# bostoncleek/ergodic_exploration

Hardware: AMD Instinct MI355X
Metric: receding-horizon optimisations/sec at K=10x10, T=200; 1/2/4/8-GPU agent-batch (higher is better)
Workload: dtype f64; 1 GPU; BASELINE configs[3]: 4096-agent batch per GPU, simple_cart, two-Gaussian 12x6 m map, K=10x10, T=200 steps (dt 0.1, horizon 20), n_mem=0; agents_per_gpu=4096, num_basis=10, horizon_steps=200, kinematics=simple_cart, agent_groups=2, steps_per_launch=50, parallelism=agent-batch x1

## Files before the change

### ergodic_exploration_amd/csrc/control_wave_impl.hpp

```cpp
#ifndef EEA_CONTROL_WAVE_HELPERS_HPP
#define EEA_CONTROL_WAVE_HELPERS_HPP

#include <type_traits>

#include "common.hpp"

#ifndef EEA_WSTAMP
#define EEA_WSTAMP(n) ((void)0)
#define EEA_WSTAMP_RT(n) ((void)0)
#define EEA_WSTAMP_HWID(n) ((void)0)
#endif

namespace eea
{
namespace wave
{
constexpr int kMaxS = 4;
constexpr int kStageRows = 32;
constexpr int kRow1 = 68;
constexpr int kTailScratch = 24;

__host__ __device__ constexpr int tab_stride(int K) { return (K + 1) & ~1; }
__host__ __device__ constexpr int park_elems() { return 2 * kMaxS * kWave; }
__host__ __device__ constexpr int d_elems(int K) { return (K * K + 3) & ~3; }
__host__ __device__ constexpr int tile_elems(int K)
// ... 118 lines not shown
{
  if constexpr (NB == 3) {
    asm volatile("s_waitcnt lgkmcnt(0)" : "+v"(qa[0]), "+v"(qa[1]), "+v"(qa[2]), "+v"(qb[0]), "+v"(qb[1]), "+v"(qb[2]));
  } else {
    static_assert(NB == 2, "lean packed instances: K = 5 or 10");
    asm volatile("s_waitcnt lgkmcnt(0)" : "+v"(qa[0]), "+v"(qa[1]), "+v"(qb[0]), "+v"(qb[1]));
  }
}

template <int N>
__device__ __forceinline__ double add_row_ror(double v)
{
  return v + dpp_or_zero<0x120 + N, 0xf>(v);
}

template <typename R, int MODEL>
__device__ __forceinline__ void model_xy(R vx, R vy, R c, R s, R& fx, R& fy)
{
  if (MODEL == kModelOmni) {
    fx = vx * c - vy * s;
    fy = vx * s + vy * c;
  } else {
    fx = vx * c;
    fy = vx * s;
  }
}

template <typename R>
__device__ __forceinline__ R wrap_pi_fast(R rad)
{
  const R pi = static_cast<R>(kPi), two_pi = static_cast<R>(2.0 * kPi);
  const R q = floor((rad + pi) * static_cast<R>(1.0 / (2.0 * kPi)));
  rad = (rad + pi) - q * two_pi;
  if (rad < R(0)) rad += two_pi;
  if (rad >= two_pi) rad -= two_pi;
  return rad - pi;
}

constexpr int waves_per_simd(int KC, int real_size)
{
  return (KC == 20) ? (real_size == 8 ? 2 : 4) : ((KC <= 10 || real_size == 4) ? 4 : 3);
}
constexpr int grad_block(int KC) { return KC; }

}
}
#endif

namespace eea
{
namespace wave
{
template <typename R, int MODEL, int KC, bool STAGES, int WPB, bool RESIDENT = false>
__global__ __launch_bounds__(WPB* kWave, waves_per_simd(KC, sizeof(R))) void control_wave_kernel(
    const ControlParams<R> p_arg, const unsigned B, const int S_arg, const int rollout_arg)
{
  (void)p_arg;
  extern __shared__ __attribute__((aligned(16))) char smem_raw[];
// ... 195 lines not shown
      sincospi_r(th_pre0 * inv_pi, &s, &c);
    }
    bool small = true;
#pragma unroll
    for (int j = 0; j < kMaxS; ++j) small = small && (fabs(dt * (R(0.5) * w[j]) * inv_pi) <= R(0.0625));
    const bool fast_h = sizeof(R) == 8 && __all(small);
    R rx = R(0), ry = R(0);
#pragma unroll
    for (int j = 0; j < kMaxS; ++j) {
      incx[j] = incy[j] = R(0);
      if (j < S) {
        R sm_, cm, cpost, spost;
        if (fast_h) {
          R sd, cd;
          sincospi_small(dt * (R(0.5) * w[j]) * inv_pi, &sd, &cd);
          cm = c * cd - s * sd;
          sm_ = s * cd + c * sd;
          cpost = cm * cd - sm_ * sd;
          spost = sm_ * cd + cm * sd;
        } else {
          const R th_pre = (j == 0) ? thp[0] - dt6 * (((w[0] + R(2) * w[0]) + R(2) * w[0]) + w[0]) : thp[j - 1];
          sincospi_r((th_pre + dt * (R(0.5) * w[j])) * inv_pi, &sm_, &cm);
          const R c2m = R(1) - R(2) * sm_ * sm_, s2m = R(2) * sm_ * cm;
          cpost = c2m * c + s2m * s;
          spost = s2m * c - c2m * s;
        }
        R k1x, k1y, k2x, k2y, k4x, k4y;
        model_xy<R, MODEL>(vx[j], vy[j], c, s, k1x, k1y);
        model_xy<R, MODEL>(vx[j], vy[j], cm, sm_, k2x, k2y);
        model_xy<R, MODEL>(vx[j], vy[j], cpost, spost, k4x, k4y);
        incx[j] = dt6 * (((k1x + R(2) * k2x) + R(2) * k2x) + k4x);
        incy[j] = dt6 * (((k1y + R(2) * k2y) + R(2) * k2y) + k4y);
        rx += incx[j];
        ry += incy[j];
        s_cp[j * kWave + lane] = cpost;
        s_sp[j * kWave + lane] = spost;
        c = cpost;
        s = spost;
      }
      px[j] = rx;
      py[j] = ry;
    }
    const R ix = wave_inclusive_scan_dpp(rx), iy = wave_inclusive_scan_dpp(ry);
    const R bx = x0 + (ix - rx), by = y0 + (iy - ry);
#pragma unroll
    for (int j = 0; j < kMaxS; ++j) {
      px[j] += bx;
// ... 18 lines not shown
  R c1x[kMaxS], s1x[kMaxS], c1y[kMaxS], s1y[kMaxS], g0[kMaxS], g1[kMaxS];
  bool small_b = true;
#pragma unroll
  for (int j = 1; j < kMaxS; ++j) {
    small_b = small_b && (fabs(incx[j] * p.inv_lx) <= R(0.0625)) && (fabs(incy[j] * p.inv_ly) <= R(0.0625));
  }
  const bool fast_b = sizeof(R) == 8 && __all(small_b);
#pragma unroll
  for (int j = 0; j < kMaxS; ++j) {
    c1x[j] = s1x[j] = c1y[j] = s1y[j] = g0[j] = g1[j] = R(0);
    if (j < S) {
      const R x = px[j] - map_x, y = py[j] - map_y;
      if (j > 0 && fast_b) {
        R sd, cd;
        sincospi_small(incx[j] * p.inv_lx, &sd, &cd);
        c1x[j] = c1x[j - 1] * cd - s1x[j - 1] * sd;
        s1x[j] = s1x[j - 1] * cd + c1x[j - 1] * sd;
        sincospi_small(incy[j] * p.inv_ly, &sd, &cd);
        c1y[j] = c1y[j - 1] * cd - s1y[j - 1] * sd;
        s1y[j] = s1y[j - 1] * cd + c1y[j - 1] * sd;
      } else {
        sincospi_r(x * p.inv_lx, &s1x[j], &c1x[j]);
        sincospi_r(y * p.inv_ly, &s1y[j], &c1y[j]);
      }
      const R eps = R(0.05), weight2 = R(50);
      g0[j] = (fmax(x - (p.lx - eps), R(0)) + fmin(x - eps, R(0))) * weight2;
      g1[j] = (fmax(y - (p.ly - eps), R(0)) + fmin(y - eps, R(0))) * weight2;
    }
  }

  EEA_WSTAMP(4);
  int nmem = 0;
  if (p.mem_cols != nullptr) {
    nmem = RESIDENT ? res_nmem : (p.n_mem != nullptr) ? p.n_mem[b] : static_cast<int>(p.mem_stride);
    nmem = nmem < 0 ? 0 : (nmem > static_cast<int>(p.mem_stride) ? static_cast<int>(p.mem_stride) : nmem);
// ... 510 lines not shown
    for (int t = 0; t < NT * NT; ++t) {
#pragma unroll
      for (int r = 0; r < 4; ++r) {
        const int k1 = 16 * (t / NT) + M::row(lane, r);
        const int k2 = 16 * (t % NT) + mi;
        if (k1 < K && k2 < K) {
          R c = invN * (*accs[t])[r];
          if (use_shared) c = shared_ck_value(p, shared_ck, ck_shared_step, k2 * K + k1, c);
          s_D[k2 * K + k1] = lam[t][r] * (c - phi[t][r]);
        }
      }
    }
    lds_fence();
  }

  EEA_WSTAMP(6);
  constexpr int KA = (KC == 16) ? 16 : KC;
  if (!STAGES) {
#pragma unroll
    for (int j = 0; j < kMaxS; ++j) {
      if (j < S) {
        s_g[(2 * j + 0) * kWave + lane] = g0[j];
        s_g[(2 * j + 1) * kWave + lane] = g1[j];
      }
    }
  }
  R ex[STAGES ? kMaxS : 1], ey[STAGES ? kMaxS : 1];
  constexpr bool kCoopTail = sizeof(R) == 8 && (KC == 10 || KC == 5);
  const bool coop_tail = kCoopTail && top_heavy && S == kMaxS;
  constexpr bool kPairGrad = sizeof(R) == 4 && (KC == 20 || KC == 10);
  if constexpr (kPairGrad) {
    typedef float f2 __attribute__((ext_vector_type(2)));
    auto splat = [](float v) { return f2{ v, v }; };
    int zoff = 0;
    asm volatile("" : "+s"(zoff));
    const R* const s_Dz = s_D + zoff;
    auto d_pair = [&](int k2, int k1) { return *reinterpret_cast<const f2*>(((k1 & 2) ? s_Dz : s_D) + k2 * K + k1); };
#pragma unroll
    for (int jp = 0; jp < kMaxS; jp += 2) {
      if (STAGES) ex[jp] = ey[jp] = ex[jp + 1] = ey[jp + 1] = R(0);
      asm volatile("" ::: "memory");
      __builtin_amdgcn_sched_barrier(0);
// ... 67 lines not shown
              ex[j] = exj;
              ey[j] = eyj;
            } else {
              const bool act = j < cnt;
              g0[j] = act ? exj + s_g[(2 * j + 0) * kWave + lane] : R(0);
              g1[j] = act ? eyj + s_g[(2 * j + 1) * kWave + lane] : R(0);
            }
          }
        }
      }
    }
  }
#pragma unroll
  for (int j = 0; j < kMaxS; ++j) {
    if (kPairGrad) break;
    if (STAGES) ex[j] = ey[j] = R(0);
    asm volatile("" ::: "memory");
    __builtin_amdgcn_sched_barrier(0);
    if (j < S && !(j == kMaxS - 1 && coop_tail)) {
      constexpr int KB = grad_block(KC);
      R accx = R(0), accy = R(0);
      const R twox = c1x[j] + c1x[j], twoy = c1y[j] + c1y[j];
      R ta = R(1), tb = c1x[j];
      R ua = R(0), ub = R(1);
#pragma unroll
      for (int kb0 = 0; kb0 < KA; kb0 += KB) {
        if (kb0 > 0) {
          asm volatile("" ::: "memory");
          __builtin_amdgcn_sched_barrier(0);
        }
        R cxa[KB], G[KB];
#pragma unroll
        for (int i = 0; i < KB; ++i) {
          cxa[i] = ta;
          const R tn = twox * tb - ta;
          ta = tb;
          tb = tn;
        }
        {
        {
          const R* const row = s_D + kb0;
#pragma unroll
          for (int i = 0; i < KB; ++i) {
            const int k1 = kb0 + i;
            G[i] = (k1 == 0 || k1 >= KA) ? R(0) : ((kGenericK && k1 >= K) ? R(0) : row[i]);
          }
        }
        R um = R(0), u0 = R(1);
        R tm = R(1), t0 = c1y[j];
#pragma unroll
        for (int k2 = 1; k2 < KA; ++k2) {
          if (!kRowGuard || k2 < K) {
            const R* const row = s_D + k2 * K + kb0;
            R h = R(0);
// ... 17 lines not shown
          }
        }
        }
#pragma unroll
        for (int i = 0; i < KB; ++i) {
          const int k1 = kb0 + i;
          if (k1 > 0 && k1 < KA) accx = fma_k(ua * G[i], k1, accx);
          const R un = twox * ub - ua;
          ua = ub;
          ub = un;
        }
      }
      const R sx = s1x[j], sy = s1y[j];
      const R exj = (-p.pi_lx * sx * accx) * p.expl_weight;
      const R eyj = (-p.pi_ly * sy * accy) * p.expl_weight;
      if (STAGES) {
        ex[j] = exj;
        ey[j] = eyj;
      } else {
        const bool act = j < cnt;
        g0[j] = act ? exj + s_g[(2 * j + 0) * kWave + lane] : R(0);
        g1[j] = act ? eyj + s_g[(2 * j + 1) * kWave + lane] : R(0);
      }
    }
  }
  if constexpr (kCoopTail) {
    if (coop_tail) {
      constexpr int jt = kMaxS - 1;
      asm volatile("" ::: "memory");
      __builtin_amdgcn_sched_barrier(0);
      const int st = lane >> 3, sub = lane & 7;
      R* const s_tail = s_g + 2 * kMaxS * kWave;
      if (lane < 8) {
        s_tail[lane] = c1x[jt];
        s_tail[8 + lane] = c1y[jt];
        s_tail[16 + lane] = s1y[jt];
      }
// ... 58 lines not shown
      px += dpp_or_zero<0xB1, 0xf>(px);
      py += dpp_or_zero<0xB1, 0xf>(py);
      px += dpp_or_zero<0x4E, 0xf>(px);
      py += dpp_or_zero<0x4E, 0xf>(py);
      px += dpp_or_zero<0x141, 0xf>(px);
      py += dpp_or_zero<0x141, 0xf>(py);
      if (sub == 0) {
        s_tail[2 * st] = px;
        s_tail[2 * st + 1] = py;
      }
      lds_fence();
      const R accx = s_tail[2 * (lane & 7)], accy = s_tail[2 * (lane & 7) + 1];
      const R sx = s1x[jt];
      const R exj = (-p.pi_lx * sx * accx) * p.expl_weight;
      const R eyj = (-p.pi_ly * accy) * p.expl_weight;
      if (STAGES) {
        ex[jt] = exj;
        ey[jt] = eyj;
      } else {
        const bool act = jt < cnt;
        g0[jt] = act ? exj + s_g[(2 * jt + 0) * kWave + lane] : R(0);
        g1[jt] = act ? eyj + s_g[(2 * jt + 1) * kWave + lane] : R(0);
      }
    }
  }
  if (STAGES) {
#pragma unroll
    for (int j = 0; j < kMaxS; ++j) {
      if (j < cnt) {
        if (p.edx != nullptr) {
          R* const o = p.edx + 3 * (static_cast<size_t>(T) * b + i0 + j);
          o[0] = ex[j];
          o[1] = ey[j];
          o[2] = R(0);
        }
        if (p.bdx != nullptr) {
          R* const o = p.bdx + 3 * (static_cast<size_t>(T) * b + i0 + j);
          o[0] = g0[j];
          o[1] = g1[j];
          o[2] = R(0);
        }
      }
    }
  }

  EEA_WSTAMP(7);
  R vxr[kMaxS], vyr[kMaxS];
  {
    size_t opaque = 0;
    asm volatile("" : "+v"(opaque));
    const R* const ut_again = ut + opaque;
#pragma unroll
    for (int j = 0; j < kMaxS; ++j) {
      const int src = i0 + j + 1;
      const bool ok = j < cnt && src < T;
      const int idx = ok ? 3 * src : 0;
      const R a = ut_again[idx];
      vxr[j] = ok ? a : R(0);
      vyr[j] = R(0);
      if (MODEL == kModelOmni) {
        const R bq = ut_again[idx + 1];
        vyr[j] = ok ? bq : R(0);
      }
    }
  }
  R r0[kMaxS], r1[kMaxS];
  R tot0, tot1, tot2;
  {
    R s0 = R(0), s1 = R(0);
#pragma unroll
    for (int j = kMaxS - 1; j >= 0; --j) {
      if (STAGES) {
        const bool act = j < cnt;
        g0[j] = act ? ex[j] + g0[j] : R(0);
        g1[j] = act ? ey[j] + g1[j] : R(0);
      }
      s0 += dt * g0[j];
      s1 += dt * g1[j];
      r0[j] = s0;
      r1[j] = s1;
    }
    const R i0s = wave_inclusive_scan_dpp(s0), i1s = wave_inclusive_scan_dpp(s1);
    tot0 = read_lane63(i0s);
    tot1 = read_lane63(i1s);
    const R o0 = tot0 - i0s, o1 = tot1 - i1s;
#pragma unroll
    for (int j = 0; j < kMaxS; ++j) {
// ... 103 lines not shown
```

Measured before the change: 182.0 million optimisations/s.

## Hold D coefficient matrix in registers and broadcast via DPP in gradient

For f64 with K=10 or 5, the Fourier coefficient matrix D is loaded once from LDS into a few VGPRs per lane. The per-step gradient contraction then reads it through hand-written v_fmac_f64_dpp row_newbcast assembly instead of repeated LDS row reads. The edx/bdx stores are also moved into the per-slot loop, and explicit FMA helpers are applied to the RK4 rotation and basis recurrences. The aim is to cut LDS traffic and latency in the gradient loop, at the cost of extra registers, fragile inline asm with manual s_nop hazards, and slightly different rounding from the FMAs.

```diff
diff --git a/ergodic_exploration_amd/csrc/control_wave_impl.hpp b/ergodic_exploration_amd/csrc/control_wave_impl.hpp
--- a/ergodic_exploration_amd/csrc/control_wave_impl.hpp
+++ b/ergodic_exploration_amd/csrc/control_wave_impl.hpp
@@ -9,6 +9,9 @@
 #define EEA_WSTAMP(n) ((void)0)
 #define EEA_WSTAMP_RT(n) ((void)0)
 #define EEA_WSTAMP_HWID(n) ((void)0)
+#endif
+#ifndef EEA_WAVE_REGD
+#define EEA_WAVE_REGD 1
 #endif
 
 namespace eea
@@ -157,6 +160,19 @@
   return v + dpp_or_zero<0x120 + N, 0xf>(v);
 }
 
+template <typename R>
+__device__ __forceinline__ R mul_sub(R a, R b, R c, R d)
+{
+  if constexpr (sizeof(R) == 8) return __builtin_fma(a, b, -(c * d));
+  else return a * b - c * d;
+}
+template <typename R>
+__device__ __forceinline__ R mul_add(R a, R b, R c, R d)
+{
+  if constexpr (sizeof(R) == 8) return __builtin_fma(a, b, c * d);
+  else return a * b + c * d;
+}
+
 template <typename R, int MODEL>
 __device__ __forceinline__ void model_xy(R vx, R vy, R c, R s, R& fx, R& fy)
 {
@@ -168,6 +184,29 @@
     fy = vx * s;
   }
 }
+template <int MODEL>
+__device__ __forceinline__ void model_xy_pinned(double vx, double vy, double c, double s, double& fx, double& fy)
+{
+  if (MODEL == kModelOmni) {
+    fx = mul_sub(vx, c, vy, s);
+    fy = mul_add(vx, s, vy, c);
+  } else {
+    fx = vx * c;
+    fy = vx * s;
+  }
+}
+template <int MODEL>
+__device__ __forceinline__ void model_xy_plus(double vx, double vy, double c, double s, double ax, double ay, double& fx,
+                                              double& fy)
+{
+  if (MODEL == kModelOmni) {
+    fx = mul_sub(vx, c, vy, s) + ax;
+    fy = mul_add(vx, s, vy, c) + ay;
+  } else {
+    fx = __builtin_fma(vx, c, ax);
+    fy = __builtin_fma(vx, s, ay);
+  }
+}
 
 template <typename R>
 __device__ __forceinline__ R wrap_pi_fast(R rad)
@@ -185,6 +224,8 @@
   return (KC == 20) ? (real_size == 8 ? 2 : 4) : ((KC <= 10 || real_size == 4) ? 4 : 3);
 }
 constexpr int grad_block(int KC) { return KC; }
+
+#include "control_wave_regd.inc"
 
 }
 }
@@ -410,23 +451,32 @@
         if (fast_h) {
           R sd, cd;
           sincospi_small(dt * (R(0.5) * w[j]) * inv_pi, &sd, &cd);
-          cm = c * cd - s * sd;
-          sm_ = s * cd + c * sd;
-          cpost = cm * cd - sm_ * sd;
-          spost = sm_ * cd + cm * sd;
+          cm = mul_sub(c, cd, s, sd);
+          sm_ = mul_add(c, sd, s, cd);
+          cpost = mul_sub(cm, cd, sm_, sd);
+          spost = mul_add(sm_, cd, cm, sd);
         } else {
           const R th_pre = (j == 0) ? thp[0] - dt6 * (((w[0] + R(2) * w[0]) + R(2) * w[0]) + w[0]) : thp[j - 1];
           sincospi_r((th_pre + dt * (R(0.5) * w[j])) * inv_pi, &sm_, &cm);
           const R c2m = R(1) - R(2) * sm_ * sm_, s2m = R(2) * sm_ * cm;
-          cpost = c2m * c + s2m * s;
-          spost = s2m * c - c2m * s;
-        }
-        R k1x, k1y, k2x, k2y, k4x, k4y;
-        model_xy<R, MODEL>(vx[j], vy[j], c, s, k1x, k1y);
-        model_xy<R, MODEL>(vx[j], vy[j], cm, sm_, k2x, k2y);
-        model_xy<R, MODEL>(vx[j], vy[j], cpost, spost, k4x, k4y);
-        incx[j] = dt6 * (((k1x + R(2) * k2x) + R(2) * k2x) + k4x);
-        incy[j] = dt6 * (((k1y + R(2) * k2y) + R(2) * k2y) + k4y);
+          cpost = mul_add(s2m, s, c2m, c);
+          spost = mul_sub(s2m, c, c2m, s);
+        }
+        if constexpr (sizeof(R) == 8) {
+          double k2x, k2y, k4x, k4y, k12x, k12y;
+          model_xy_pinned<MODEL>(vx[j], vy[j], cm, sm_, k2x, k2y);
+          model_xy_pinned<MODEL>(vx[j], vy[j], cpost, spost, k4x, k4y);
+          model_xy_plus<MODEL>(vx[j], vy[j], c, s, k2x + k2x, k2y + k2y, k12x, k12y);
+          incx[j] = dt6 * ((k12x + R(2) * k2x) + k4x);
+          incy[j] = dt6 * ((k12y + R(2) * k2y) + k4y);
+        } else {
+          R k1x, k1y, k2x, k2y, k4x, k4y;
+          model_xy<R, MODEL>(vx[j], vy[j], c, s, k1x, k1y);
+          model_xy<R, MODEL>(vx[j], vy[j], cm, sm_, k2x, k2y);
+          model_xy<R, MODEL>(vx[j], vy[j], cpost, spost, k4x, k4y);
+          incx[j] = dt6 * (((k1x + R(2) * k2x) + R(2) * k2x) + k4x);
+          incy[j] = dt6 * (((k1y + R(2) * k2y) + R(2) * k2y) + k4y);
+        }
         rx += incx[j];
         ry += incy[j];
         s_cp[j * kWave + lane] = cpost;
@@ -475,11 +525,12 @@
       if (j > 0 && fast_b) {
         R sd, cd;
         sincospi_small(incx[j] * p.inv_lx, &sd, &cd);
-        c1x[j] = c1x[j - 1] * cd - s1x[j - 1] * sd;
-        s1x[j] = s1x[j - 1] * cd + c1x[j - 1] * sd;
+        constexpr bool kFuseSCdX = (KC == 20), kFuseSCdY = (KC == 20 || KC == 5);
+        c1x[j] = mul_sub(c1x[j - 1], cd, s1x[j - 1], sd);
+        s1x[j] = kFuseSCdX ? mul_add(s1x[j - 1], cd, c1x[j - 1], sd) : mul_add(c1x[j - 1], sd, s1x[j - 1], cd);
         sincospi_small(incy[j] * p.inv_ly, &sd, &cd);
-        c1y[j] = c1y[j - 1] * cd - s1y[j - 1] * sd;
-        s1y[j] = s1y[j - 1] * cd + c1y[j - 1] * sd;
+        c1y[j] = mul_sub(c1y[j - 1], cd, s1y[j - 1], sd);
+        s1y[j] = kFuseSCdY ? mul_add(s1y[j - 1], cd, c1y[j - 1], sd) : mul_add(c1y[j - 1], sd, s1y[j - 1], cd);
       } else {
         sincospi_r(x * p.inv_lx, &s1x[j], &c1x[j]);
         sincospi_r(y * p.inv_ly, &s1y[j], &c1y[j]);
@@ -1020,9 +1071,34 @@
     lds_fence();
   }
 
+  constexpr bool kRegD = EEA_WAVE_REGD && sizeof(R) == 8 && (KC == 10 || KC == 5);
+  constexpr int kDRegs = kRegD ? (KC * KC + 15) / 16 : 1;
+  double Dv[kDRegs];
+  if constexpr (kRegD) {
+#pragma unroll
+    for (int q = 0; q < kDRegs; ++q) Dv[q] = s_D[min(16 * q + (lane & 15), KC * KC - 1)];
+  }
+
   EEA_WSTAMP(6);
   constexpr int KA = (KC == 16) ? 16 : KC;
-  if (!STAGES) {
+  constexpr bool kSumInSlot = !STAGES || kRegD;
+  auto store_edx_bdx = [&](int j, R exj, R eyj, R bx, R by) {
+    if (j < cnt) {
+      if (p.edx != nullptr) {
+        R* const o = p.edx + 3 * (static_cast<size_t>(T) * b + i0 + j);
+        o[0] = exj;
+        o[1] = eyj;
+        o[2] = R(0);
+      }
+      if (p.bdx != nullptr) {
+        R* const o = p.bdx + 3 * (static_cast<size_t>(T) * b + i0 + j);
+        o[0] = bx;
+        o[1] = by;
+        o[2] = R(0);
+      }
+    }
+  };
+  if (kSumInSlot) {
 #pragma unroll
     for (int j = 0; j < kMaxS; ++j) {
       if (j < S) {
@@ -1031,7 +1107,7 @@
       }
     }
   }
-  R ex[STAGES ? kMaxS : 1], ey[STAGES ? kMaxS : 1];
+  R ex[kSumInSlot ? 1 : kMaxS], ey[kSumInSlot ? 1 : kMaxS];
   constexpr bool kCoopTail = sizeof(R) == 8 && (KC == 10 || KC == 5);
   const bool coop_tail = kCoopTail && top_heavy && S == kMaxS;
   constexpr bool kPairGrad = sizeof(R) == 4 && (KC == 20 || KC == 10);
@@ -1129,7 +1205,7 @@
 #pragma unroll
   for (int j = 0; j < kMaxS; ++j) {
     if (kPairGrad) break;
-    if (STAGES) ex[j] = ey[j] = R(0);
+    if (!kSumInSlot) ex[j] = ey[j] = R(0);
     asm volatile("" ::: "memory");
     __builtin_amdgcn_sched_barrier(0);
     if (j < S && !(j == kMaxS - 1 && coop_tail)) {
@@ -1152,7 +1228,9 @@
           ta = tb;
           tb = tn;
         }
-        {
+        if constexpr (kRegD) {
+          RegDGrad<kRegD ? KC : 5>::run(Dv, cxa, G, c1y[j], twoy, accy);
+        } else {
         {
           const R* const row = s_D + kb0;
 #pragma unroll
@@ -1200,13 +1278,15 @@
       const R sx = s1x[j], sy = s1y[j];
       const R exj = (-p.pi_lx * sx * accx) * p.expl_weight;
       const R eyj = (-p.pi_ly * sy * accy) * p.expl_weight;
-      if (STAGES) {
+      if (!kSumInSlot) {
         ex[j] = exj;
         ey[j] = eyj;
       } else {
         const bool act = j < cnt;
-        g0[j] = act ? exj + s_g[(2 * j + 0) * kWave + lane] : R(0);
-        g1[j] = act ? eyj + s_g[(2 * j + 1) * kWave + lane] : R(0);
+        const R bx = s_g[(2 * j + 0) * kWave + lane], by = s_g[(2 * j + 1) * kWave + lane];
+        if (STAGES) store_edx_bdx(j, exj, eyj, bx, by);
+        g0[j] = act ? exj + bx : R(0);
+        g1[j] = act ? eyj + by : R(0);
       }
     }
   }
@@ -1295,34 +1375,21 @@
       const R sx = s1x[jt];
       const R exj = (-p.pi_lx * sx * accx) * p.expl_weight;
       const R eyj = (-p.pi_ly * accy) * p.expl_weight;
-      if (STAGES) {
+      if (!kSumInSlot) {
         ex[jt] = exj;
         ey[jt] = eyj;
       } else {
         const bool act = jt < cnt;
-        g0[jt] = act ? exj + s_g[(2 * jt + 0) * kWave + lane] : R(0);
-        g1[jt] = act ? eyj + s_g[(2 * jt + 1) * kWave + lane] : R(0);
-      }
-    }
-  }
-  if (STAGES) {
-#pragma unroll
-    for (int j = 0; j < kMaxS; ++j) {
-      if (j < cnt) {
-        if (p.edx != nullptr) {
-          R* const o = p.edx + 3 * (static_cast<size_t>(T) * b + i0 + j);
-          o[0] = ex[j];
-          o[1] = ey[j];
-          o[2] = R(0);
-        }
-        if (p.bdx != nullptr) {
-          R* const o = p.bdx + 3 * (static_cast<size_t>(T) * b + i0 + j);
-          o[0] = g0[j];
-          o[1] = g1[j];
-          o[2] = R(0);
-        }
-      }
-    }
+        const R bx = s_g[(2 * jt + 0) * kWave + lane], by = s_g[(2 * jt + 1) * kWave + lane];
+        if (STAGES) store_edx_bdx(jt, exj, eyj, bx, by);
+        g0[jt] = act ? exj + bx : R(0);
+        g1[jt] = act ? eyj + by : R(0);
+      }
+    }
+  }
+  if (STAGES && !kSumInSlot) {
+#pragma unroll
+    for (int j = 0; j < kMaxS; ++j) store_edx_bdx(j, ex[j], ey[j], g0[j], g1[j]);
   }
 
   EEA_WSTAMP(7);
@@ -1351,7 +1418,7 @@
     R s0 = R(0), s1 = R(0);
 #pragma unroll
     for (int j = kMaxS - 1; j >= 0; --j) {
-      if (STAGES) {
+      if (!kSumInSlot) {
         const bool act = j < cnt;
         g0[j] = act ? ex[j] + g0[j] : R(0);
         g1[j] = act ? ey[j] + g1[j] : R(0);
diff --git a/ergodic_exploration_amd/csrc/control_wave_regd.inc b/ergodic_exploration_amd/csrc/control_wave_regd.inc
--- /dev/null
+++ b/ergodic_exploration_amd/csrc/control_wave_regd.inc
@@ -0,0 +1,402 @@
+template <int K>
+struct RegDGrad;
+template <>
+struct RegDGrad<5>
+{
+  static constexpr int kRegs = 2;
+  static __device__ __forceinline__ void run(const double (&Dv)[2], const double (&cxa)[5], double (&G)[5],
+                                             double cy, double twoy, double& accy)
+  {
+    double um = 0.0, u0 = 1.0;
+    double tm = 1.0, t0 = cy;
+    double t1, h0, h1;
+    asm volatile(
+        "s_nop 1\n\t"
+        "v_mov_b64_dpp %[h0], %[d0] row_newbcast:5 row_mask:0xf bank_mask:0xf\n\t"
+        "v_mov_b64_dpp %[g1], %[d0] row_newbcast:1 row_mask:0xf bank_mask:0xf\n\t"
+        "v_mov_b64_dpp %[g2], %[d0] row_newbcast:2 row_mask:0xf bank_mask:0xf\n\t"
+        "v_fmac_f64_dpp %[h0], %[d0], %[c1] row_newbcast:6 row_mask:0xf bank_mask:0xf\n\t"
+        "v_mov_b64_dpp %[g3], %[d0] row_newbcast:3 row_mask:0xf bank_mask:0xf\n\t"
+        "v_mov_b64_dpp %[g4], %[d0] row_newbcast:4 row_mask:0xf bank_mask:0xf\n\t"
+        "v_fmac_f64_dpp %[h0], %[d0], %[c2] row_newbcast:7 row_mask:0xf bank_mask:0xf\n\t"
+        "v_fmac_f64_dpp %[g1], %[d0], %[t0] row_newbcast:6 row_mask:0xf bank_mask:0xf\n\t"
+        "v_fmac_f64_dpp %[g2], %[d0], %[t0] row_newbcast:7 row_mask:0xf bank_mask:0xf\n\t"
+        "v_fmac_f64_dpp %[h0], %[d0], %[c3] row_newbcast:8 row_mask:0xf bank_mask:0xf\n\t"
+        "v_fmac_f64_dpp %[g3], %[d0], %[t0] row_newbcast:8 row_mask:0xf bank_mask:0xf\n\t"
+        "v_fmac_f64_dpp %[g4], %[d0], %[t0] row_newbcast:9 row_mask:0xf bank_mask:0xf\n\t"
+        "v_fmac_f64_dpp %[h0], %[d0], %[c4] row_newbcast:9 row_mask:0xf bank_mask:0xf\n\t"
+        : [g1] "=&v"(G[1]), [g2] "=&v"(G[2]), [g3] "=&v"(G[3]), [g4] "=&v"(G[4]), [h0] "=&v"(h0)
+        : [d0] "v"(Dv[0]), [t0] "v"(t0), [c1] "v"(cxa[1]), [c2] "v"(cxa[2]), [c3] "v"(cxa[3]), [c4] "v"(cxa[4]));
+    G[0] = 0.0;
+    accy = fma_k(u0 * h0, 1, accy);
+    {
+      const double un = twoy * u0 - um;
+      um = u0;
+      u0 = un;
+    }
+    {
+      const double tn = twoy * t0 - tm;
+      tm = t0;
+      t0 = tn;
+    }
+    asm volatile("" : "+v"(t0), "+v"(tm), "+v"(u0), "+v"(um));
+    t1 = twoy * t0 - tm;
+    asm volatile(
+        "s_nop 1\n\t"
+        "v_mov_b64_dpp %[h0], %[d0] row_newbcast:10 row_mask:0xf bank_mask:0xf\n\t"
+        "v_mov_b64_dpp %[h1], %[d0] row_newbcast:15 row_mask:0xf bank_mask:0xf\n\t"
+        "v_fmac_f64_dpp %[g1], %[d0], %[t0] row_newbcast:11 row_mask:0xf bank_mask:0xf\n\t"
+        "v_fmac_f64_dpp %[h0], %[d0], %[c1] row_newbcast:11 row_mask:0xf bank_mask:0xf\n\t"
+        "v_fmac_f64_dpp %[h1], %[d1], %[c1] row_newbcast:0 row_mask:0xf bank_mask:0xf\n\t"
+        "v_fmac_f64_dpp %[g2], %[d0], %[t0] row_newbcast:12 row_mask:0xf bank_mask:0xf\n\t"
+        "v_fmac_f64_dpp %[h0], %[d0], %[c2] row_newbcast:12 row_mask:0xf bank_mask:0xf\n\t"
+        "v_fmac_f64_dpp %[h1], %[d1], %[c2] row_newbcast:1 row_mask:0xf bank_mask:0xf\n\t"
+        "v_fmac_f64_dpp %[g3], %[d0], %[t0] row_newbcast:13 row_mask:0xf bank_mask:0xf\n\t"
+        "v_fmac_f64_dpp %[h0], %[d0], %[c3] row_newbcast:13 row_mask:0xf bank_mask:0xf\n\t"
+        "v_fmac_f64_dpp %[h1], %[d1], %[c3] row_newbcast:2 row_mask:0xf bank_mask:0xf\n\t"
+        "v_fmac_f64_dpp %[g4], %[d0], %[t0] row_newbcast:14 row_mask:0xf bank_mask:0xf\n\t"
+        "v_fmac_f64_dpp %[h0], %[d0], %[c4] row_newbcast:14 row_mask:0xf bank_mask:0xf\n\t"
+        "v_fmac_f64_dpp %[h1], %[d1], %[c4] row_newbcast:3 row_mask:0xf bank_mask:0xf\n\t"
+        "v_fmac_f64_dpp %[g1], %[d1], %[t1] row_newbcast:0 row_mask:0xf bank_mask:0xf\n\t"
+        "v_fmac_f64_dpp %[g2], %[d1], %[t1] row_newbcast:1 row_mask:0xf bank_mask:0xf\n\t"
+        "v_fmac_f64_dpp %[g3], %[d1], %[t1] row_newbcast:2 row_mask:0xf bank_mask:0xf\n\t"
+        "v_fmac_f64_dpp %[g4], %[d1], %[t1] row_newbcast:3 row_mask:0xf bank_mask:0xf\n\t"
+        : [g1] "+v"(G[1]), [g2] "+v"(G[2]), [g3] "+v"(G[3]), [g4] "+v"(G[4]), [h0] "=&v"(h0), [h1] "=&v"(h1)
+        : [d0] "v"(Dv[0]), [d1] "v"(Dv[1]), [t0] "v"(t0), [t1] "v"(t1), [c1] "v"(cxa[1]), [c2] "v"(cxa[2]), [c3] "v"(cxa[3]), [c4] "v"(cxa[4]));
+    accy = fma_k(u0 * h0, 2, accy);
+    {
+      const double un = twoy * u0 - um;
+      um = u0;
+      u0 = un;
+    }
+    accy = fma_k(u0 * h1, 3, accy);
+    {
+      const double un = twoy * u0 - um;
+      um = u0;
+      u0 = un;
+    }
+    tm = t1;
+    t0 = twoy * t1 - t0;
+    asm volatile("" : "+v"(t0), "+v"(tm), "+v"(u0), "+v"(um));
+    asm volatile(
+        "s_nop 1\n\t"
+        "v_mov_b64_dpp %[h0], %[d1] row_newbcast:4 row_mask:0xf bank_mask:0xf\n\t"
+        "v_fmac_f64_dpp %[g1], %[d1], %[t0] row_newbcast:5 row_mask:0xf bank_mask:0xf\n\t"
+        "v_fmac_f64_dpp %[g2], %[d1], %[t0] row_newbcast:6 row_mask:0xf bank_mask:0xf\n\t"
+        "v_fmac_f64_dpp %[h0], %[d1], %[c1] row_newbcast:5 row_mask:0xf bank_mask:0xf\n\t"
+        "v_fmac_f64_dpp %[g3], %[d1], %[t0] row_newbcast:7 row_mask:0xf bank_mask:0xf\n\t"
+        "v_fmac_f64_dpp %[g4], %[d1], %[t0] row_newbcast:8 row_mask:0xf bank_mask:0xf\n\t"
+        "v_fmac_f64_dpp %[h0], %[d1], %[c2] row_newbcast:6 row_mask:0xf bank_mask:0xf\n\t"
+        "s_nop 1\n\t"
+        "v_fmac_f64_dpp %[h0], %[d1], %[c3] row_newbcast:7 row_mask:0xf bank_mask:0xf\n\t"
+        "s_nop 1\n\t"
+        "v_fmac_f64_dpp %[h0], %[d1], %[c4] row_newbcast:8 row_mask:0xf bank_mask:0xf\n\t"
+        : [g1] "+v"(G[1]), [g2] "+v"(G[2]), [g3] "+v"(G[3]), [g4] "+v"(G[4]), [h0] "=&v"(h0)
+        : [d1] "v"(Dv[1]), [t0] "v"(t0), [c1] "v"(cxa[1]), [c2] "v"(cxa[2]), [c3] "v"(cxa[3]), [c4] "v"(cxa[4]));
+    accy = fma_k(u0 * h0, 4, accy);
+    {
+      const double un = twoy * u0 - um;
+      um = u0;
+      u0 = un;
+    }
+    {
+      const double tn = twoy * t0 - tm;
+      tm = t0;
+      t0 = tn;
+    }
+    asm volatile("" : "+v"(t0), "+v"(tm), "+v"(u0), "+v"(um));
+    (void)t1;
+    (void)h1;
+  }
+};
+template <>
+struct RegDGrad<10>
+{
+  static constexpr int kRegs = 7;
+  static __device__ __forceinline__ void run(const double (&Dv)[7], const double (&cxa)[10], double (&G)[10],
+                                             double cy, double twoy, double& accy)
+  {
+    double um = 0.0, u0 = 1.0;
+    double tm = 1.0, t0 = cy;
+    double t1, h0, h1;
+    asm volatile(
+        "s_nop 1\n\t"
+        "v_mov_b64_dpp %[h0], %[d0] row_newbcast:10 row_mask:0xf bank_mask:0xf\n\t"
+        "v_mov_b64_dpp %[g1], %[d0] row_newbcast:1 row_mask:0xf bank_mask:0xf\n\t"
+        "v_mov_b64_dpp %[g2], %[d0] row_newbcast:2 row_mask:0xf bank_mask:0xf\n\t"
+        "v_fmac_f64_dpp %[h0], %[d0], %[c1] row_newbcast:11 row_mask:0xf bank_mask:0xf\n\t"
+        "v_mov_b64_dpp %[g3], %[d0] row_newbcast:3 row_mask:0xf bank_mask:0xf\n\t"
+        "v_mov_b64_dpp %[g4], %[d0] row_newbcast:4 row_mask:0xf bank_mask:0xf\n\t"
+        "v_fmac_f64_dpp %[h0], %[d0], %[c2] row_newbcast:12 row_mask:0xf bank_mask:0xf\n\t"
+        "v_mov_b64_dpp %[g5], %[d0] row_newbcast:5 row_mask:0xf bank_mask:0xf\n\t"
+        "v_mov_b64_dpp %[g6], %[d0] row_newbcast:6 row_mask:0xf bank_mask:0xf\n\t"
+        "v_fmac_f64_dpp %[h0], %[d0], %[c3] row_newbcast:13 row_mask:0xf bank_mask:0xf\n\t"
+        "v_mov_b64_dpp %[g7], %[d0] row_newbcast:7 row_mask:0xf bank_mask:0xf\n\t"
+        "v_mov_b64_dpp %[g8], %[d0] row_newbcast:8 row_mask:0xf bank_mask:0xf\n\t"
+        "v_fmac_f64_dpp %[h0], %[d0], %[c4] row_newbcast:14 row_mask:0xf bank_mask:0xf\n\t"
+        "v_mov_b64_dpp %[g9], %[d0] row_newbcast:9 row_mask:0xf bank_mask:0xf\n\t"
+        "v_fmac_f64_dpp %[g1], %[d0], %[t0] row_newbcast:11 row_mask:0xf bank_mask:0xf\n\t"
+        "v_fmac_f64_dpp %[h0], %[d0], %[c5] row_newbcast:15 row_mask:0xf bank_mask:0xf\n\t"
+        "v_fmac_f64_dpp %[g2], %[d0], %[t0] row_newbcast:12 row_mask:0xf bank_mask:0xf\n\t"
+        "v_fmac_f64_dpp %[g3], %[d0], %[t0] row_newbcast:13 row_mask:0xf bank_mask:0xf\n\t"
+        "v_fmac_f64_dpp %[h0], %[d1], %[c6] row_newbcast:0 row_mask:0xf bank_mask:0xf\n\t"
+        "v_fmac_f64_dpp %[g4], %[d0], %[t0] row_newbcast:14 row_mask:0xf bank_mask:0xf\n\t"
+        "v_fmac_f64_dpp %[g5], %[d0], %[t0] row_newbcast:15 row_mask:0xf bank_mask:0xf\n\t"
+        "v_fmac_f64_dpp %[h0], %[d1], %[c7] row_newbcast:1 row_mask:0xf bank_mask:0xf\n\t"
+        "v_fmac_f64_dpp %[g6], %[d1], %[t0] row_newbcast:0 row_mask:0xf bank_mask:0xf\n\t"
+        "v_fmac_f64_dpp %[g7], %[d1], %[t0] row_newbcast:1 row_mask:0xf bank_mask:0xf\n\t"
+        "v_fmac_f64_dpp %[h0], %[d1], %[c8] row_newbcast:2 row_mask:0xf bank_mask:0xf\n\t"
+        "v_fmac_f64_dpp %[g8], %[d1], %[t0] row_newbcast:2 row_mask:0xf bank_mask:0xf\n\t"
+        "v_fmac_f64_dpp %[g9], %[d1], %[t0] row_newbcast:3 row_mask:0xf bank_mask:0xf\n\t"
+        "v_fmac_f64_dpp %[h0], %[d1], %[c9] row_newbcast:3 row_mask:0xf bank_mask:0xf\n\t"
+        : [g1] "=&v"(G[1]), [g2] "=&v"(G[2]), [g3] "=&v"(G[3]), [g4] "=&v"(G[4]), [g5] "=&v"(G[5]), [g6] "=&v"(G[6]), [g7] "=&v"(G[7]), [g8] "=&v"(G[8]), [g9] "=&v"(G[9]), [h0] "=&v"(h0)
+        : [d0] "v"(Dv[0]), [d1] "v"(Dv[1]), [t0] "v"(t0), [c1] "v"(cxa[1]), [c2] "v"(cxa[2]), [c3] "v"(cxa[3]), [c4] "v"(cxa[4]), [c5] "v"(cxa[5]), [c6] "v"(cxa[6]), [c7] "v"(cxa[7]), [c8] "v"(cxa[8]), [c9] "v"(cxa[9]));
+    G[0] = 0.0;
+    accy = fma_k(u0 * h0, 1, accy);
+    {
+      const double un = twoy * u0 - um;
+      um = u0;
+      u0 = un;
+    }
+    {
+      const double tn = twoy * t0 - tm;
+      tm = t0;
+      t0 = tn;
+    }
+    asm volatile("" : "+v"(t0), "+v"(tm), "+v"(u0), "+v"(um));
+    t1 = twoy * t0 - tm;
+    asm volatile(
+        "s_nop 1\n\t"
+        "v_mov_b64_dpp %[h0], %[d1] row_newbcast:4 row_mask:0xf bank_mask:0xf\n\t"
+        "v_mov_b64_dpp %[h1], %[d1] row_newbcast:14 row_mask:0xf bank_mask:0xf\n\t"
+        "v_fmac_f64_dpp %[g1], %[d1], %[t0] row_newbcast:5 row_mask:0xf bank_mask:0xf\n\t"
+        "v_fmac_f64_dpp %[h0], %[d1], %[c1] row_newbcast:5 row_mask:0xf bank_mask:0xf\n\t"
+        "v_fmac_f64_dpp %[h1], %[d1], %[c1] row_newbcast:15 row_mask:0xf bank_mask:0xf\n\t"
+        "v_fmac_f64_dpp %[g2], %[d1], %[t0] row_newbcast:6 row_mask:0xf bank_mask:0xf\n\t"
+        "v_fmac_f64_dpp %[h0], %[d1], %[c2] row_newbcast:6 row_mask:0xf bank_mask:0xf\n\t"
+        "v_fmac_f64_dpp %[h1], %[d2], %[c2] row_newbcast:0 row_mask:0xf bank_mask:0xf\n\t"
+        "v_fmac_f64_dpp %[g3], %[d1], %[t0] row_newbcast:7 row_mask:0xf bank_mask:0xf\n\t"
+        "v_fmac_f64_dpp %[h0], %[d1], %[c3] row_newbcast:7 row_mask:0xf bank_mask:0xf\n\t"
+        "v_fmac_f64_dpp %[h1], %[d2], %[c3] row_newbcast:1 row_mask:0xf bank_mask:0xf\n\t"
+        "v_fmac_f64_dpp %[g4], %[d1], %[t0] row_newbcast:8 row_mask:0xf bank_mask:0xf\n\t"
+        "v_fmac_f64_dpp %[h0], %[d1], %[c4] row_newbcast:8 row_mask:0xf bank_mask:0xf\n\t"
+        "v_fmac_f64_dpp %[h1], %[d2], %[c4] row_newbcast:2 row_mask:0xf bank_mask:0xf\n\t"
+        "v_fmac_f64_dpp %[g5], %[d1], %[t0] row_newbcast:9 row_mask:0xf bank_mask:0xf\n\t"
+        "v_fmac_f64_dpp %[h0], %[d1], %[c5] row_newbcast:9 row_mask:0xf bank_mask:0xf\n\t"
+        "v_fmac_f64_dpp %[h1], %[d2], %[c5] row_newbcast:3 row_mask:0xf bank_mask:0xf\n\t"
+        "v_fmac_f64_dpp %[g6], %[d1], %[t0] row_newbcast:10 row_mask:0xf bank_mask:0xf\n\t"
+        "v_fmac_f64_dpp %[h0], %[d1], %[c6] row_newbcast:10 row_mask:0xf bank_mask:0xf\n\t"
+        "v_fmac_f64_dpp %[h1], %[d2], %[c6] row_newbcast:4 row_mask:0xf bank_mask:0xf\n\t"
+        "v_fmac_f64_dpp %[g7], %[d1], %[t0] row_newbcast:11 row_mask:0xf bank_mask:0xf\n\t"
+        "v_fmac_f64_dpp %[h0], %[d1], %[c7] row_newbcast:11 row_mask:0xf bank_mask:0xf\n\t"
+        "v_fmac_f64_dpp %[h1], %[d2], %[c7] row_newbcast:5 row_mask:0xf bank_mask:0xf\n\t"
+        "v_fmac_f64_dpp %[g8], %[d1], %[t0] row_newbcast:12 row_mask:0xf bank_mask:0xf\n\t"
+        "v_fmac_f64_dpp %[h0], %[d1], %[c8] row_newbcast:12 row_mask:0xf bank_mask:0xf\n\t"
+        "v_fmac_f64_dpp %[h1], %[d2], %[c8] row_newbcast:6 row_mask:0xf bank_mask:0xf\n\t"
+        "v_fmac_f64_dpp %[g9], %[d1], %[t0] row_newbcast:13 row_mask:0xf bank_mask:0xf\n\t"
+        "v_fmac_f64_dpp %[h0], %[d1], %[c9] row_newbcast:13 row_mask:0xf bank_mask:0xf\n\t"
+        "v_fmac_f64_dpp %[h1], %[d2], %[c9] row_newbcast:7 row_mask:0xf bank_mask:0xf\n\t"
+        "v_fmac_f64_dpp %[g1], %[d1], %[t1] row_newbcast:15 row_mask:0xf bank_mask:0xf\n\t"
+        "v_fmac_f64_dpp %[g2], %[d2], %[t1] row_newbcast:0 row_mask:0xf bank_mask:0xf\n\t"
+        "v_fmac_f64_dpp %[g3], %[d2], %[t1] row_newbcast:1 row_mask:0xf bank_mask:0xf\n\t"
+        "v_fmac_f64_dpp %[g4], %[d2], %[t1] row_newbcast:2 row_mask:0xf bank_mask:0xf\n\t"
+        "v_fmac_f64_dpp %[g5], %[d2], %[t1] row_newbcast:3 row_mask:0xf bank_mask:0xf\n\t"
+        "v_fmac_f64_dpp %[g6], %[d2], %[t1] row_newbcast:4 row_mask:0xf bank_mask:0xf\n\t"
+        "v_fmac_f64_dpp %[g7], %[d2], %[t1] row_newbcast:5 row_mask:0xf bank_mask:0xf\n\t"
+        "v_fmac_f64_dpp %[g8], %[d2], %[t1] row_newbcast:6 row_mask:0xf bank_mask:0xf\n\t"
+        "v_fmac_f64_dpp %[g9], %[d2], %[t1] row_newbcast:7 row_mask:0xf bank_mask:0xf\n\t"
+        : [g1] "+v"(G[1]), [g2] "+v"(G[2]), [g3] "+v"(G[3]), [g4] "+v"(G[4]), [g5] "+v"(G[5]), [g6] "+v"(G[6]), [g7] "+v"(G[7]), [g8] "+v"(G[8]), [g9] "+v"(G[9]), [h0] "=&v"(h0), [h1] "=&v"(h1)
+        : [d1] "v"(Dv[1]), [d2] "v"(Dv[2]), [t0] "v"(t0), [t1] "v"(t1), [c1] "v"(cxa[1]), [c2] "v"(cxa[2]), [c3] "v"(cxa[3]), [c4] "v"(cxa[4]), [c5] "v"(cxa[5]), [c6] "v"(cxa[6]), [c7] "v"(cxa[7]), [c8] "v"(cxa[8]), [c9] "v"(cxa[9]));
+    accy = fma_k(u0 * h0, 2, accy);
+    {
+      const double un = twoy * u0 - um;
+      um = u0;
+      u0 = un;
+    }
+    accy = fma_k(u0 * h1, 3, accy);
+    {
+      const double un = twoy * u0 - um;
+      um = u0;
+      u0 = un;
+    }
+    tm = t1;
+    t0 = twoy * t1 - t0;
+    asm volatile("" : "+v"(t0), "+v"(tm), "+v"(u0), "+v"(um));
+    t1 = twoy * t0 - tm;
+    asm volatile(
+        "s_nop 1\n\t"
+        "v_mov_b64_dpp %[h0], %[d2] row_newbcast:8 row_mask:0xf bank_mask:0xf\n\t"
+        "v_mov_b64_dpp %[h1], %[d3] row_newbcast:2 row_mask:0xf bank_mask:0xf\n\t"
+        "v_fmac_f64_dpp %[g1], %[d2], %[t0] row_newbcast:9 row_mask:0xf bank_mask:0xf\n\t"
+        "v_fmac_f64_dpp %[h0], %[d2], %[c1] row_newbcast:9 row_mask:0xf bank_mask:0xf\n\t"
+        "v_fmac_f64_dpp %[h1], %[d3], %[c1] row_newbcast:3 row_mask:0xf bank_mask:0xf\n\t"
+        "v_fmac_f64_dpp %[g2], %[d2], %[t0] row_newbcast:10 row_mask:0xf bank_mask:0xf\n\t"
+        "v_fmac_f64_dpp %[h0], %[d2], %[c2] row_newbcast:10 row_mask:0xf bank_mask:0xf\n\t"
+        "v_fmac_f64_dpp %[h1], %[d3], %[c2] row_newbcast:4 row_mask:0xf bank_mask:0xf\n\t"
+        "v_fmac_f64_dpp %[g3], %[d2], %[t0] row_newbcast:11 row_mask:0xf bank_mask:0xf\n\t"
+        "v_fmac_f64_dpp %[h0], %[d2], %[c3] row_newbcast:11 row_mask:0xf bank_mask:0xf\n\t"
+        "v_fmac_f64_dpp %[h1], %[d3], %[c3] row_newbcast:5 row_mask:0xf bank_mask:0xf\n\t"
+        "v_fmac_f64_dpp %[g4], %[d2], %[t0] row_newbcast:12 row_mask:0xf bank_mask:0xf\n\t"
+        "v_fmac_f64_dpp %[h0], %[d2], %[c4] row_newbcast:12 row_mask:0xf bank_mask:0xf\n\t"
+        "v_fmac_f64_dpp %[h1], %[d3], %[c4] row_newbcast:6 row_mask:0xf bank_mask:0xf\n\t"
+        "v_fmac_f64_dpp %[g5], %[d2], %[t0] row_newbcast:13 row_mask:0xf bank_mask:0xf\n\t"
+        "v_fmac_f64_dpp %[h0], %[d2], %[c5] row_newbcast:13 row_mask:0xf bank_mask:0xf\n\t"
+        "v_fmac_f64_dpp %[h1], %[d3], %[c5] row_newbcast:7 row_mask:0xf bank_mask:0xf\n\t"
+        "v_fmac_f64_dpp %[g6], %[d2], %[t0] row_newbcast:14 row_mask:0xf bank_mask:0xf\n\t"
+        "v_fmac_f64_dpp %[h0], %[d2], %[c6] row_newbcast:14 row_mask:0xf bank_mask:0xf\n\t"
+        "v_fmac_f64_dpp %[h1], %[d3], %[c6] row_newbcast:8 row_mask:0xf bank_mask:0xf\n\t"
+        "v_fmac_f64_dpp %[g7], %[d2], %[t0] row_newbcast:15 row_mask:0xf bank_mask:0xf\n\t"
+        "v_fmac_f64_dpp %[h0], %[d2], %[c7] row_newbcast:15 row_mask:0xf bank_mask:0xf\n\t"
+        "v_fmac_f64_dpp %[h1], %[d3], %[c7] row_newbcast:9 row_mask:0xf bank_mask:0xf\n\t"
+        "v_fmac_f64_dpp %[g8], %[d3], %[t0] row_newbcast:0 row_mask:0xf bank_mask:0xf\n\t"
+        "v_fmac_f64_dpp %[h0], %[d3], %[c8] row_newbcast:0 row_mask:0xf bank_mask:0xf\n\t"
+        "v_fmac_f64_dpp %[h1], %[d3], %[c8] row_newbcast:10 row_mask:0xf bank_mask:0xf\n\t"
+        "v_fmac_f64_dpp %[g9], %[d3], %[t0] row_newbcast:1 row_mask:0xf bank_mask:0xf\n\t"
+        "v_fmac_f64_dpp %[h0], %[d3], %[c9] row_newbcast:1 row_mask:0xf bank_mask:0xf\n\t"
+        "v_fmac_f64_dpp %[h1], %[d3], %[c9] row_newbcast:11 row_mask:0xf bank_mask:0xf\n\t"
+        "v_fmac_f64_dpp %[g1], %[d3], %[t1] row_newbcast:3 row_mask:0xf bank_mask:0xf\n\t"
+        "v_fmac_f64_dpp %[g2], %[d3], %[t1] row_newbcast:4 row_mask:0xf bank_mask:0xf\n\t"
+        "v_fmac_f64_dpp %[g3], %[d3], %[t1] row_newbcast:5 row_mask:0xf bank_mask:0xf\n\t"
+        "v_fmac_f64_dpp %[g4], %[d3], %[t1] row_newbcast:6 row_mask:0xf bank_mask:0xf\n\t"
+        "v_fmac_f64_dpp %[g5], %[d3], %[t1] row_newbcast:7 row_mask:0xf bank_mask:0xf\n\t"
+        "v_fmac_f64_dpp %[g6], %[d3], %[t1] row_newbcast:8 row_mask:0xf bank_mask:0xf\n\t"
+        "v_fmac_f64_dpp %[g7], %[d3], %[t1] row_newbcast:9 row_mask:0xf bank_mask:0xf\n\t"
+        "v_fmac_f64_dpp %[g8], %[d3], %[t1] row_newbcast:10 row_mask:0xf bank_mask:0xf\n\t"
+        "v_fmac_f64_dpp %[g9], %[d3], %[t1] row_newbcast:11 row_mask:0xf bank_mask:0xf\n\t"
+        : [g1] "+v"(G[1]), [g2] "+v"(G[2]), [g3] "+v"(G[3]), [g4] "+v"(G[4]), [g5] "+v"(G[5]), [g6] "+v"(G[6]), [g7] "+v"(G[7]), [g8] "+v"(G[8]), [g9] "+v"(G[9]), [h0] "=&v"(h0), [h1] "=&v"(h1)
+        : [d2] "v"(Dv[2]), [d3] "v"(Dv[3]), [t0] "v"(t0), [t1] "v"(t1), [c1] "v"(cxa[1]), [c2] "v"(cxa[2]), [c3] "v"(cxa[3]), [c4] "v"(cxa[4]), [c5] "v"(cxa[5]), [c6] "v"(cxa[6]), [c7] "v"(cxa[7]), [c8] "v"(cxa[8]), [c9] "v"(cxa[9]));
+    accy = fma_k(u0 * h0, 4, accy);
+    {
+      const double un = twoy * u0 - um;
+      um = u0;
+      u0 = un;
+    }
+    accy = fma_k(u0 * h1, 5, accy);
+    {
+      const double un = twoy * u0 - um;
+      um = u0;
+      u0 = un;
+    }
+    tm = t1;
+    t0 = twoy * t1 - t0;
+    asm volatile("" : "+v"(t0), "+v"(tm), "+v"(u0), "+v"(um));
+    t1 = twoy * t0 - tm;
+    asm volatile(
+        "s_nop 1\n\t"
+        "v_mov_b64_dpp %[h0], %[d3] row_newbcast:12 row_mask:0xf bank_mask:0xf\n\t"
+        "v_mov_b64_dpp %[h1], %[d4] row_newbcast:6 row_mask:0xf bank_mask:0xf\n\t"
+        "v_fmac_f64_dpp %[g1], %[d3], %[t0] row_newbcast:13 row_mask:0xf bank_mask:0xf\n\t"
+        "v_fmac_f64_dpp %[h0], %[d3], %[c1] row_newbcast:13 row_mask:0xf bank_mask:0xf\n\t"
+        "v_fmac_f64_dpp %[h1], %[d4], %[c1] row_newbcast:7 row_mask:0xf bank_mask:0xf\n\t"
+        "v_fmac_f64_dpp %[g2], %[d3], %[t0] row_newbcast:14 row_mask:0xf bank_mask:0xf\n\t"
+        "v_fmac_f64_dpp %[h0], %[d3], %[c2] row_newbcast:14 row_mask:0xf bank_mask:0xf\n\t"
+        "v_fmac_f64_dpp %[h1], %[d4], %[c2] row_newbcast:8 row_mask:0xf bank_mask:0xf\n\t"
+        "v_fmac_f64_dpp %[g3], %[d3], %[t0] row_newbcast:15 row_mask:0xf bank_mask:0xf\n\t"
+        "v_fmac_f64_dpp %[h0], %[d3], %[c3] row_newbcast:15 row_mask:0xf bank_mask:0xf\n\t"
+        "v_fmac_f64_dpp %[h1], %[d4], %[c3] row_newbcast:9 row_mask:0xf bank_mask:0xf\n\t"
+        "v_fmac_f64_dpp %[g4], %[d4], %[t0] row_newbcast:0 row_mask:0xf bank_mask:0xf\n\t"
+        "v_fmac_f64_dpp %[h0], %[d4], %[c4] row_newbcast:0 row_mask:0xf bank_mask:0xf\n\t"
+        "v_fmac_f64_dpp %[h1], %[d4], %[c4] row_newbcast:10 row_mask:0xf bank_mask:0xf\n\t"
+        "v_fmac_f64_dpp %[g5], %[d4], %[t0] row_newbcast:1 row_mask:0xf bank_mask:0xf\n\t"
+        "v_fmac_f64_dpp %[h0], %[d4], %[c5] row_newbcast:1 row_mask:0xf bank_mask:0xf\n\t"
+        "v_fmac_f64_dpp %[h1], %[d4], %[c5] row_newbcast:11 row_mask:0xf bank_mask:0xf\n\t"
+        "v_fmac_f64_dpp %[g6], %[d4], %[t0] row_newbcast:2 row_mask:0xf bank_mask:0xf\n\t"
+        "v_fmac_f64_dpp %[h0], %[d4], %[c6] row_newbcast:2 row_mask:0xf bank_mask:0xf\n\t"
+        "v_fmac_f64_dpp %[h1], %[d4], %[c6] row_newbcast:12 row_mask:0xf bank_mask:0xf\n\t"
+        "v_fmac_f64_dpp %[g7], %[d4], %[t0] row_newbcast:3 row_mask:0xf bank_mask:0xf\n\t"
+        "v_fmac_f64_dpp %[h0], %[d4], %[c7] row_newbcast:3 row_mask:0xf bank_mask:0xf\n\t"
+        "v_fmac_f64_dpp %[h1], %[d4], %[c7] row_newbcast:13 row_mask:0xf bank_mask:0xf\n\t"
+        "v_fmac_f64_dpp %[g8], %[d4], %[t0] row_newbcast:4 row_mask:0xf bank_mask:0xf\n\t"
+        "v_fmac_f64_dpp %[h0], %[d4], %[c8] row_newbcast:4 row_mask:0xf bank_mask:0xf\n\t"
+        "v_fmac_f64_dpp %[h1], %[d4], %[c8] row_newbcast:14 row_mask:0xf bank_mask:0xf\n\t"
+        "v_fmac_f64_dpp %[g9], %[d4], %[t0] row_newbcast:5 row_mask:0xf bank_mask:0xf\n\t"
+        "v_fmac_f64_dpp %[h0], %[d4], %[c9] row_newbcast:5 row_mask:0xf bank_mask:0xf\n\t"
+        "v_fmac_f64_dpp %[h1], %[d4], %[c9] row_newbcast:15 row_mask:0xf bank_mask:0xf\n\t"
+        "v_fmac_f64_dpp %[g1], %[d4], %[t1] row_newbcast:7 row_mask:0xf bank_mask:0xf\n\t"
+        "v_fmac_f64_dpp %[g2], %[d4], %[t1] row_newbcast:8 row_mask:0xf bank_mask:0xf\n\t"
+        "v_fmac_f64_dpp %[g3], %[d4], %[t1] row_newbcast:9 row_mask:0xf bank_mask:0xf\n\t"
+        "v_fmac_f64_dpp %[g4], %[d4], %[t1] row_newbcast:10 row_mask:0xf bank_mask:0xf\n\t"
+        "v_fmac_f64_dpp %[g5], %[d4], %[t1] row_newbcast:11 row_mask:0xf bank_mask:0xf\n\t"
+        "v_fmac_f64_dpp %[g6], %[d4], %[t1] row_newbcast:12 row_mask:0xf bank_mask:0xf\n\t"
+        "v_fmac_f64_dpp %[g7], %[d4], %[t1] row_newbcast:13 row_mask:0xf bank_mask:0xf\n\t"
+        "v_fmac_f64_dpp %[g8], %[d4], %[t1] row_newbcast:14 row_mask:0xf bank_mask:0xf\n\t"
+        "v_fmac_f64_dpp %[g9], %[d4], %[t1] row_newbcast:15 row_mask:0xf bank_mask:0xf\n\t"
+        : [g1] "+v"(G[1]), [g2] "+v"(G[2]), [g3] "+v"(G[3]), [g4] "+v"(G[4]), [g5] "+v"(G[5]), [g6] "+v"(G[6]), [g7] "+v"(G[7]), [g8] "+v"(G[8]), [g9] "+v"(G[9]), [h0] "=&v"(h0), [h1] "=&v"(h1)
+        : [d3] "v"(Dv[3]), [d4] "v"(Dv[4]), [t0] "v"(t0), [t1] "v"(t1), [c1] "v"(cxa[1]), [c2] "v"(cxa[2]), [c3] "v"(cxa[3]), [c4] "v"(cxa[4]), [c5] "v"(cxa[5]), [c6] "v"(cxa[6]), [c7] "v"(cxa[7]), [c8] "v"(cxa[8]), [c9] "v"(cxa[9]));
+    accy = fma_k(u0 * h0, 6, accy);
+    {
+      const double un = twoy * u0 - um;
+      um = u0;
+      u0 = un;
+    }
+    accy = fma_k(u0 * h1, 7, accy);
+    {
+      const double un = twoy * u0 - um;
+      um = u0;
+      u0 = un;
+    }
+    tm = t1;
+    t0 = twoy * t1 - t0;
+    asm volatile("" : "+v"(t0), "+v"(tm), "+v"(u0), "+v"(um));
+    t1 = twoy * t0 - tm;
+    asm volatile(
+        "s_nop 1\n\t"
+        "v_mov_b64_dpp %[h0], %[d5] row_newbcast:0 row_mask:0xf bank_mask:0xf\n\t"
+        "v_mov_b64_dpp %[h1], %[d5] row_newbcast:10 row_mask:0xf bank_mask:0xf\n\t"
+        "v_fmac_f64_dpp %[g1], %[d5], %[t0] row_newbcast:1 row_mask:0xf bank_mask:0xf\n\t"
+        "v_fmac_f64_dpp %[h0], %[d5], %[c1] row_newbcast:1 row_mask:0xf bank_mask:0xf\n\t"
+        "v_fmac_f64_dpp %[h1], %[d5], %[c1] row_newbcast:11 row_mask:0xf bank_mask:0xf\n\t"
+        "v_fmac_f64_dpp %[g2], %[d5], %[t0] row_newbcast:2 row_mask:0xf bank_mask:0xf\n\t"
+        "v_fmac_f64_dpp %[h0], %[d5], %[c2] row_newbcast:2 row_mask:0xf bank_mask:0xf\n\t"
+        "v_fmac_f64_dpp %[h1], %[d5], %[c2] row_newbcast:12 row_mask:0xf bank_mask:0xf\n\t"
+        "v_fmac_f64_dpp %[g3], %[d5], %[t0] row_newbcast:3 row_mask:0xf bank_mask:0xf\n\t"
+        "v_fmac_f64_dpp %[h0], %[d5], %[c3] row_newbcast:3 row_mask:0xf bank_mask:0xf\n\t"
+        "v_fmac_f64_dpp %[h1], %[d5], %[c3] row_newbcast:13 row_mask:0xf bank_mask:0xf\n\t"
+        "v_fmac_f64_dpp %[g4], %[d5], %[t0] row_newbcast:4 row_mask:0xf bank_mask:0xf\n\t"
+        "v_fmac_f64_dpp %[h0], %[d5], %[c4] row_newbcast:4 row_mask:0xf bank_mask:0xf\n\t"
+        "v_fmac_f64_dpp %[h1], %[d5], %[c4] row_newbcast:14 row_mask:0xf bank_mask:0xf\n\t"
+        "v_fmac_f64_dpp %[g5], %[d5], %[t0] row_newbcast:5 row_mask:0xf bank_mask:0xf\n\t"
+        "v_fmac_f64_dpp %[h0], %[d5], %[c5] row_newbcast:5 row_mask:0xf bank_mask:0xf\n\t"
+        "v_fmac_f64_dpp %[h1], %[d5], %[c5] row_newbcast:15 row_mask:0xf bank_mask:0xf\n\t"
+        "v_fmac_f64_dpp %[g6], %[d5], %[t0] row_newbcast:6 row_mask:0xf bank_mask:0xf\n\t"
+        "v_fmac_f64_dpp %[h0], %[d5], %[c6] row_newbcast:6 row_mask:0xf bank_mask:0xf\n\t"
+        "v_fmac_f64_dpp %[h1], %[d6], %[c6] row_newbcast:0 row_mask:0xf bank_mask:0xf\n\t"
+        "v_fmac_f64_dpp %[g7], %[d5], %[t0] row_newbcast:7 row_mask:0xf bank_mask:0xf\n\t"
+        "v_fmac_f64_dpp %[h0], %[d5], %[c7] row_newbcast:7 row_mask:0xf bank_mask:0xf\n\t"
+        "v_fmac_f64_dpp %[h1], %[d6], %[c7] row_newbcast:1 row_mask:0xf bank_mask:0xf\n\t"
+        "v_fmac_f64_dpp %[g8], %[d5], %[t0] row_newbcast:8 row_mask:0xf bank_mask:0xf\n\t"
+        "v_fmac_f64_dpp %[h0], %[d5], %[c8] row_newbcast:8 row_mask:0xf bank_mask:0xf\n\t"
+        "v_fmac_f64_dpp %[h1], %[d6], %[c8] row_newbcast:2 row_mask:0xf bank_mask:0xf\n\t"
+        "v_fmac_f64_dpp %[g9], %[d5], %[t0] row_newbcast:9 row_mask:0xf bank_mask:0xf\n\t"
+        "v_fmac_f64_dpp %[h0], %[d5], %[c9] row_newbcast:9 row_mask:0xf bank_mask:0xf\n\t"
+        "v_fmac_f64_dpp %[h1], %[d6], %[c9] row_newbcast:3 row_mask:0xf bank_mask:0xf\n\t"
+        "v_fmac_f64_dpp %[g1], %[d5], %[t1] row_newbcast:11 row_mask:0xf bank_mask:0xf\n\t"
+        "v_fmac_f64_dpp %[g2], %[d5], %[t1] row_newbcast:12 row_mask:0xf bank_mask:0xf\n\t"
+        "v_fmac_f64_dpp %[g3], %[d5], %[t1] row_newbcast:13 row_mask:0xf bank_mask:0xf\n\t"
+        "v_fmac_f64_dpp %[g4], %[d5], %[t1] row_newbcast:14 row_mask:0xf bank_mask:0xf\n\t"
+        "v_fmac_f64_dpp %[g5], %[d5], %[t1] row_newbcast:15 row_mask:0xf bank_mask:0xf\n\t"
+        "v_fmac_f64_dpp %[g6], %[d6], %[t1] row_newbcast:0 row_mask:0xf bank_mask:0xf\n\t"
+        "v_fmac_f64_dpp %[g7], %[d6], %[t1] row_newbcast:1 row_mask:0xf bank_mask:0xf\n\t"
+        "v_fmac_f64_dpp %[g8], %[d6], %[t1] row_newbcast:2 row_mask:0xf bank_mask:0xf\n\t"
+        "v_fmac_f64_dpp %[g9], %[d6], %[t1] row_newbcast:3 row_mask:0xf bank_mask:0xf\n\t"
+        : [g1] "+v"(G[1]), [g2] "+v"(G[2]), [g3] "+v"(G[3]), [g4] "+v"(G[4]), [g5] "+v"(G[5]), [g6] "+v"(G[6]), [g7] "+v"(G[7]), [g8] "+v"(G[8]), [g9] "+v"(G[9]), [h0] "=&v"(h0), [h1] "=&v"(h1)
+        : [d5] "v"(Dv[5]), [d6] "v"(Dv[6]), [t0] "v"(t0), [t1] "v"(t1), [c1] "v"(cxa[1]), [c2] "v"(cxa[2]), [c3] "v"(cxa[3]), [c4] "v"(cxa[4]), [c5] "v"(cxa[5]), [c6] "v"(cxa[6]), [c7] "v"(cxa[7]), [c8] "v"(cxa[8]), [c9] "v"(cxa[9]));
+    accy = fma_k(u0 * h0, 8, accy);
+    {
+      const double un = twoy * u0 - um;
+      um = u0;
+      u0 = un;
+    }
+    accy = fma_k(u0 * h1, 9, accy);
+    {
+      const double un = twoy * u0 - um;
+      um = u0;
+      u0 = un;
+    }
+    tm = t1;
+    t0 = twoy * t1 - t0;
+    asm volatile("" : "+v"(t0), "+v"(tm), "+v"(u0), "+v"(um));
+    (void)t1;
+    (void)h1;
+  }
+};
```

Result: faster. 190.1 million optimisations/s, median of 6 (+4.4%).
